# ajgupta93/d4pg-pytorch

Hardware: AMD Instinct MI355X
Metric: learner grad-steps/sec (Pendulum-v1 D4PG) (higher is better)
Workload: dtype fp32; 1 GPU; model=D4PG Pendulum-v1 (obs3/act1, 4x256 MLP actor+critic, 51 atoms), global_batch=64, parallelism=dp1 (one learner per GPU), n_step=5, prioritized_replay=True, replay_capacity=1000000, device=cuda

## Files before the change

d4pg_amd/ops/hip/engine_common.hip:

```cpp

#include <hip/hip_runtime.h>
#include <cstdint>
#include <cstdio>
#include <cstring>
#include <cstdlib>
#include <cmath>
#include <vector>
#include <stdexcept>

#define HIP_CHECK(cmd) do { \
    hipError_t e_ = (cmd); \
    if (e_ != hipSuccess) { \
        char buf[256]; \
        snprintf(buf, sizeof(buf), "HIP error %s at %s:%d", \
                 hipGetErrorString(e_), __FILE__, __LINE__); \
        throw std::runtime_error(buf); \
    } \
} while (0)

namespace d4pg {

__device__ __forceinline__ uint32_t mulhi32(uint32_t a, uint32_t b) {
    return (uint32_t)(((uint64_t)a * b) >> 32);
}

struct Philox4 { uint32_t v[4]; };

__device__ inline Philox4 philox4(uint64_t seed, uint64_t ctr_hi,
                                  uint64_t ctr_lo) {
    uint32_t c0 = (uint32_t)ctr_lo, c1 = (uint32_t)(ctr_lo >> 32);
    uint32_t c2 = (uint32_t)ctr_hi, c3 = (uint32_t)(ctr_hi >> 32);
    uint32_t k0 = (uint32_t)seed, k1 = (uint32_t)(seed >> 32);
    const uint32_t M0 = 0xD2511F53u, M1 = 0xCD9E8D57u;
    const uint32_t W0 = 0x9E3779B9u, W1 = 0xBB67AE85u;
#pragma unroll
    for (int r = 0; r < 10; ++r) {
        uint32_t hi0 = mulhi32(M0, c0), lo0 = M0 * c0;
        uint32_t hi1 = mulhi32(M1, c2), lo1 = M1 * c2;
        uint32_t n0 = hi1 ^ c1 ^ k0, n1 = lo1;
        uint32_t n2 = hi0 ^ c3 ^ k1, n3 = lo0;
        c0 = n0; c1 = n1; c2 = n2; c3 = n3;
        k0 += W0; k1 += W1;
    }
    return {c0, c1, c2, c3};
}

__device__ inline float u01(uint32_t x) {
    return ((float)x + 1.0f) * 2.3283064e-10f;
}


struct LayerDesc {
    int in1, in2, out;
    long w_off, b_off;
};

enum Act { ACT_NONE = 0, ACT_RELU = 1, ACT_TANH = 2, ACT_SOFTMAX = 3 };

struct EngineCfg {
    int obs, act, hidden, atoms, batch;
    long capacity;
    float v_min, v_max, gamma_n, tau, lr_actor, lr_critic;
    float per_alpha, per_beta0, per_eps;
    long per_beta_iters;
    uint64_t seed;
    int is_weighting;
    int prioritized = 1;
    int true_td = 0;
};

struct Counters {
    long long beta_t;
    long long adam_t_actor;
    long long adam_t_critic;
    long long rng_epoch;
    long long size;
    long long pos;
    float max_priority;
    float loss_critic;
    float loss_actor;
};

#define FWD_XMAX 1032

__device__ inline float act_mask(int act, float h) {
    if (act == ACT_RELU) return h > 0.f ? 1.f : 0.f;
    if (act == ACT_TANH) return 1.f - h * h;
    return 1.f;
}

struct NetPtrs { const float *w1, *b1, *w2, *b2, *w3, *b3, *w4, *b4; };

__device__ inline NetPtrs net_ptrs(const float* slab, const LayerDesc* l) {
    return {slab + l[0].w_off, slab + l[0].b_off,
            slab + l[1].w_off, slab + l[1].b_off,
            slab + l[2].w_off, slab + l[2].b_off,
            slab + l[3].w_off, slab + l[3].b_off};
}

struct StepArgs {
    int B, O, A, H, K;
    float v_min, v_max, gamma_n, per_eps, tau, lr_actor, lr_critic;
    float per_alpha, per_beta0, per_beta_iters;
    int is_weighting;
    int prioritized, true_td;
    uint64_t seed;
    long tree_cap;
    long n_actor, n_critic;
    LayerDesc al[4], cl[4];
    float *p_actor, *p_actor_t, *p_critic, *p_critic_t;
    float *g_actor, *g_critic, *m_actor, *v_actor, *m_critic, *v_critic;
    float *rs, *ra, *rr, *rs2, *rd;
    double *sum_tree, *min_tree;
    float *bs, *bs_b, *ba, *br, *bs2, *bd, *bw, *pri;
    long *bidx;
    float *at_h1, *at_h2, *at_h3, *a2;
    float *ct_h1, *ct_h2, *ct_h3, *p_t, *m_proj;
    float *c_h1, *c_h2, *c_h3, *q, *dlog, *d3, *d2, *d1;
    float *pa_h1, *pa_h2, *pa_h3, *a_out;
    float *pc_h1, *pc_h2, *pc_h3, *pq;
    float *pd3, *pd2, *pdh1, *adz, *az1, *az2, *az3;
    Counters* cnt;
    unsigned long long* gbar;
    unsigned long long* tstamp;
    float *da, *pda;
};


}
```

d4pg_amd/ops/hip/engine_persistent.hip:

```cpp

namespace d4pg {

#define PNWG 96
#define PW4 (PNWG / 4)
#define PW3A (PNWG / 3)
#define PW3B (PNWG - 2 * (PNWG / 3))
#define PROWS 4
#define PXMAX 512
#define PWOFF (PROWS * PXMAX)
#define PLDS_FLOATS (2 * 4 * PXMAX + 2 * 64 * 68 + 64)

#define PTIMEW(g, s, i, w) \
    do { if ((int)blockIdx.x == (w) && threadIdx.x == 0 && (s) == pts) \
        (g).tstamp[i] = __builtin_amdgcn_s_memrealtime(); } while (0)
#define PTIME(g, s, i) PTIMEW(g, s, i, 0)

__device__ inline void bar_release() {
    __builtin_amdgcn_fence(__ATOMIC_RELEASE, "agent");
    asm volatile("s_waitcnt vmcnt(0)" ::: "memory");
}
__device__ inline void bar_acquire() {
    __builtin_amdgcn_fence(__ATOMIC_ACQUIRE, "agent");
    asm volatile("s_waitcnt vmcnt(0)" ::: "memory");
}

__device__ inline void p_bar(unsigned long long* gb,
                             unsigned long long& round) {
    __syncthreads();
    round += 1;
    if (threadIdx.x == 0) {
        bar_release();
        int grp = blockIdx.x & 7;
        unsigned long long old = atomicAdd(&gb[grp << 4], 1ull);
        if (old + 1 == round * (PNWG >> 3)) {
            unsigned long long r = atomicAdd(&gb[128], 1ull);
            if (r + 1 == round * 8)
                __hip_atomic_store(&gb[144], round, __ATOMIC_RELEASE,
                                   __HIP_MEMORY_SCOPE_AGENT);
        }
        volatile unsigned long long* f = &gb[144];
        volatile unsigned long long* err = &gb[176];
        long spins = 0;
        while (*f < round) {
            if (++spins > (1L << 26)) {
                atomicAdd((unsigned long long*)err, 1ull);
                break;
            }
            if (spins < 48) __builtin_amdgcn_s_sleep(2);
            else {
                __builtin_amdgcn_s_sleep(32);
                if ((spins & 63) == 0 && *err) break;
            }
        }
        bar_acquire();
    }
    __syncthreads();
}

__device__ inline void q_bar(unsigned long long* qc,
                             unsigned long long& qround) {
    __syncthreads();
    qround += 4;
    if (threadIdx.x == 0) {
        bar_release();
        atomicAdd(qc, 1ull);
        volatile unsigned long long* f = qc;
        long spins = 0;
        while (*f < qround) {
            if (++spins > (1L << 26)) break;
            __builtin_amdgcn_s_sleep(1);
        }
        bar_acquire();
    }
    __syncthreads();
}

__device__ inline void t_bar(unsigned long long* tc,
                             unsigned long long& trnd, int members) {
    __syncthreads();
    trnd += members;
    if (threadIdx.x == 0) {
        bar_release();
        atomicAdd(tc, 1ull);
        volatile unsigned long long* f = tc;
        long spins = 0;
        while (*f < trnd) {
            if (++spins > (1L << 26)) break;
            __builtin_amdgcn_s_sleep(1);
        }
        bar_acquire();
    }
    __syncthreads();
}

__device__ __noinline__ void p_fwd(float* lds, const float* x1, const float* x2,
                             const float* wt, const float* bias, float* y,
                             int B, int in1, int in2, int out, int act_kind,
                             int wg_rel, int nwg) {
    int in_total = in1 + in2;
    int in_pad = (in_total + 3) & ~3;
    int nrt = (B + PROWS - 1) / PROWS;
    int nct = (out + 63) / 64;
    int ntiles = nrt * nct;
    int tid = threadIdx.x;
    for (int t = wg_rel; t < ntiles; t += nwg) {
        int r0 = (t / nct) * PROWS, c0 = (t % nct) * 64;
        int kk16 = tid >> 6, cc16 = tid & 63;
        float wreg[16];
        int nfull = in_total >> 6;
        auto preload = [&](int kc) {
#pragma unroll
            for (int u = 0; u < 16; ++u) {
                int gk = kc + kk16 + 4 * u, gc = c0 + cc16;
                wreg[u] = (gc < out)
                    ? wt[(long)gk * out + gc] : 0.f;
            }
        };
        if (nfull > 0) preload(0);
        {
            int tot = PROWS * in_pad;
            for (int base = 0; base < tot; base += 256 * 8) {
                float tmp[8];
#pragma unroll
                for (int u = 0; u < 8; ++u) {
                    int e = base + u * 256 + tid;
                    float v = 0.f;
                    if (e < tot) {
                        int rr_ = e / in_pad, kk = e % in_pad;
                        int gb = r0 + rr_;
                        if (gb < B && kk < in_total)
                            v = (kk < in1)
                                ? x1[(long)gb * in1 + kk]
                                : x2[(long)gb * in2 + (kk - in1)];
                    }
                    tmp[u] = v;
                }
#pragma unroll
                for (int u = 0; u < 8; ++u) {
                    int e = base + u * 256 + tid;
                    if (e < tot) lds[e] = tmp[u];
                }
            }
        }
        __syncthreads();
        int rq = tid >> 6, c = tid & 63;
        int o = c0 + c;
        int r = r0 + rq;
        float acc = 0.f;
        float* ws = lds + PWOFF;
        const float* xr = lds + rq * in_pad;
        for (int ch = 0; ch < nfull; ++ch) {
            int kc = ch << 6;
            float wb[16];
#pragma unroll
            for (int u = 0; u < 16; ++u) wb[u] = wreg[u];
            if (kc + 64 < (nfull << 6)) preload(kc + 64);
#pragma unroll
            for (int u = 0; u < 16; ++u)
                ws[cc16 * 68 + kk16 + 4 * u] = wb[u];
            __syncthreads();
            if (o < out) {
                const float* wcol = ws + c * 68;
#pragma unroll
                for (int k = 0; k < 64; k += 4) {
                    float4 wv = *reinterpret_cast<const float4*>(wcol + k);
                    float4 xv = *reinterpret_cast<const float4*>(
                        xr + kc + k);
                    acc += xv.x * wv.x;
                    acc += xv.y * wv.y;
                    acc += xv.z * wv.z;
                    acc += xv.w * wv.w;
                }
            }
            __syncthreads();
        }
        int kc = nfull << 6, klen = in_total - kc;
        if (klen > 0) {
            for (int e = tid; e < (klen << 6); e += 256) {
                int kk = e >> 6, cc = e & 63;
                int gc = c0 + cc;
                ws[cc * 68 + kk] = (gc < out)
                    ? wt[(long)(kc + kk) * out + gc] : 0.f;
            }
            __syncthreads();
            if (o < out) {
                for (int k = 0; k < klen; ++k)
                    acc += xr[kc + k] * ws[c * 68 + k];
            }
            __syncthreads();
        }
        if (act_kind == ACT_SOFTMAX) {
            float v = (o < out) ? acc + bias[o] : -INFINITY;
            float mx = v;
            for (int s = 32; s > 0; s >>= 1)
                mx = fmaxf(mx, __shfl_xor(mx, s, 64));
            float e = (o < out) ? __expf(v - mx) : 0.f;
            float sum = e;
            for (int s = 32; s > 0; s >>= 1) sum += __shfl_xor(sum, s, 64);
            if (r < B && o < out) y[(long)r * out + o] = e / sum;
        } else if (r < B && o < out) {
            float v = acc + bias[o];
            if (act_kind == ACT_RELU) v = fmaxf(v, 0.f);
            else if (act_kind == ACT_TANH) v = tanhf(v);
            y[(long)r * out + o] = v;
        }
        __syncthreads();
    }
}

__device__ inline void p_bwd_dx(float* lds, const float* dz, const float* wt,
                                int in_lo, int in_hi, int out, int B,
                                const float* hprev, int prev_act, float* dx,
                                int wg_rel, int nwg) {
    int span = in_hi - in_lo;
    int nrt = (B + PROWS - 1) / PROWS;
    int nit = (span + 63) / 64;
    int ntiles = nrt * nit;
    int tid = threadIdx.x;
    for (int t = wg_rel; t < ntiles; t += nwg) {
        int r0 = (t / nit) * PROWS, i0 = in_lo + (t % nit) * 64;
        int oo16 = tid & 3;
        int ii16 = tid >> 2;
        float wreg[16];
        int gi_ld = i0 + ii16;
        int nfull = out >> 6;
        auto preload = [&](int oc) {
#pragma unroll
            for (int u = 0; u < 16; ++u) {
                int go = oc + oo16 + 4 * u;
                wreg[u] = (gi_ld < in_hi)
                    ? wt[(long)gi_ld * out + go] : 0.f;
            }
        };
        if (nfull > 0) preload(0);
        int out_pad = (out + 3) & ~3;
        {
            int tot = PROWS * out_pad;
            for (int base = 0; base < tot; base += 256 * 8) {
                float tmp[8];
#pragma unroll
                for (int u = 0; u < 8; ++u) {
                    int e = base + u * 256 + tid;
                    float v = 0.f;
                    if (e < tot) {
                        int rr_ = e / out_pad, oo = e % out_pad;
                        int gb = r0 + rr_;
                        if (gb < B && oo < out)
                            v = dz[(long)gb * out + oo];
                    }
                    tmp[u] = v;
                }
#pragma unroll
                for (int u = 0; u < 8; ++u) {
                    int e = base + u * 256 + tid;
                    if (e < tot) lds[e] = tmp[u];
                }
            }
        }
        __syncthreads();
        int rq = tid >> 6, c = tid & 63;
        int i = i0 + c;
        int r = r0 + rq;
        float acc = 0.f;
        float* ws = lds + PWOFF;
        const float* zr = lds + rq * out_pad;
        for (int ch = 0; ch < nfull; ++ch) {
            int oc = ch << 6;
            float wb[16];
#pragma unroll
            for (int u = 0; u < 16; ++u) wb[u] = wreg[u];
            if (oc + 64 < (nfull << 6)) preload(oc + 64);
#pragma unroll
            for (int u = 0; u < 16; ++u)
                ws[ii16 * 68 + oo16 + 4 * u] = wb[u];
            __syncthreads();
            if (i < in_hi) {
                const float* wrow = ws + c * 68;
#pragma unroll
                for (int o = 0; o < 64; o += 4) {
                    float4 wv = *reinterpret_cast<const float4*>(wrow + o);
                    float4 zv = *reinterpret_cast<const float4*>(
                        zr + oc + o);
                    acc += zv.x * wv.x;
                    acc += zv.y * wv.y;
                    acc += zv.z * wv.z;
                    acc += zv.w * wv.w;
                }
            }
            __syncthreads();
        }
        int oc = nfull << 6, olen = out - oc;
        if (olen > 0) {
            for (int e = tid; e < 4096; e += 256) {
                int ii = e >> 6, oo = e & 63;
                int gi = i0 + ii;
                ws[ii * 68 + oo] = (gi < in_hi && oo < olen)
                    ? wt[(long)gi * out + (oc + oo)] : 0.f;
            }
            __syncthreads();
            if (i < in_hi) {
                for (int o = 0; o < olen; ++o)
                    acc += zr[oc + o] * ws[c * 68 + o];
            }
            __syncthreads();
        }
        if (r < B && i < in_hi) {
            long rel = (long)r * span + (i - in_lo);
            float m_ = hprev ? act_mask(prev_act, hprev[rel]) : 1.f;
            dx[rel] = acc * m_;
        }
        __syncthreads();
    }
}

__device__ __noinline__ void p_dw2(float* lds, const float* dz,
                                   const float* x1, const float* x2,
                                   float* dwt, float* dbias,
                                   int B, int in1, int in2, int out,
                                   int wg_rel, int nwg) {
    int in_total = in1 + in2;
    int nti = (in_total + 63) >> 6, nto = (out + 63) >> 6;
    int ntiles = nti * nto;
    float* xs = lds;
    float* zs = lds + 64 * 68;
    int tid = threadIdx.x;
    int ig = tid >> 4, og = tid & 15;
    for (int t = wg_rel; t < ntiles; t += nwg) {
        int i0 = (t / nto) << 6, o0 = (t % nto) << 6;
        float acc[4][4] = {};
        float accb[4] = {};
        for (int bc = 0; bc < B; bc += 64) {
            float tx[16], tz[16];
#pragma unroll
            for (int u = 0; u < 16; ++u) {
                int e = u * 256 + tid;
                int bb = e >> 6, ii = e & 63;
                int gb = bc + bb, gi = i0 + ii;
                float xv = 0.f;
                if (gb < B && gi < in_total)
                    xv = (gi < in1) ? x1[(long)gb * in1 + gi]
                                    : x2[(long)gb * in2 + (gi - in1)];
                tx[u] = xv;
                int go = o0 + ii;
                tz[u] = (gb < B && go < out)
                    ? dz[(long)gb * out + go] : 0.f;
            }
#pragma unroll
            for (int u = 0; u < 16; ++u) {
                int e = u * 256 + tid;
                int bb = e >> 6, ii = e & 63;
                xs[bb * 68 + ii] = tx[u];
                zs[bb * 68 + ii] = tz[u];
            }
            __syncthreads();
            int blim = min(64, B - bc);
            for (int b = 0; b < blim; ++b) {
                float4 xq = *reinterpret_cast<const float4*>(
                    xs + b * 68 + ig * 4);
                float4 zq = *reinterpret_cast<const float4*>(
                    zs + b * 68 + og * 4);
                float xv0 = xq.x, xv1 = xq.y, xv2 = xq.z, xv3 = xq.w;
                float zv0 = zq.x, zv1 = zq.y, zv2 = zq.z, zv3 = zq.w;
                acc[0][0] += xv0 * zv0; acc[0][1] += xv0 * zv1;
                acc[0][2] += xv0 * zv2; acc[0][3] += xv0 * zv3;
                acc[1][0] += xv1 * zv0; acc[1][1] += xv1 * zv1;
                acc[1][2] += xv1 * zv2; acc[1][3] += xv1 * zv3;
                acc[2][0] += xv2 * zv0; acc[2][1] += xv2 * zv1;
                acc[2][2] += xv2 * zv2; acc[2][3] += xv2 * zv3;
                acc[3][0] += xv3 * zv0; acc[3][1] += xv3 * zv1;
                acc[3][2] += xv3 * zv2; acc[3][3] += xv3 * zv3;
                if (ig == 0 && i0 == 0) {
                    accb[0] += zv0; accb[1] += zv1;
                    accb[2] += zv2; accb[3] += zv3;
                }
            }
            __syncthreads();
        }
#pragma unroll
        for (int a = 0; a < 4; ++a) {
            int gi = i0 + ig * 4 + a;
            if (gi >= in_total) continue;
#pragma unroll
            for (int bb = 0; bb < 4; ++bb) {
                int go = o0 + og * 4 + bb;
                if (go < out) dwt[(long)gi * out + go] = acc[a][bb];
            }
        }
        if (ig == 0 && i0 == 0 && dbias) {
#pragma unroll
            for (int bb = 0; bb < 4; ++bb) {
                int go = o0 + og * 4 + bb;
                if (go < out) dbias[go] = accb[bb];
            }
        }
    }
}

__device__ inline void p_adam_lerp(float* __restrict__ p,
                                   const float* __restrict__ gr,
                                   float* __restrict__ m,
                                   float* __restrict__ v,
                                   float* __restrict__ tgt_slab, long n,
                                   float lr, float tau, long long t,
                                   int nwg = PNWG) {
    const float b1 = 0.9f, b2 = 0.999f, eps = 1e-8f;
    AdamBias bc = adam_bias(b1, b2, t);
    long stride = (long)nwg * 256;
    long i0 = (long)blockIdx.x * 256 + threadIdx.x;
    for (long base = i0; base < n; base += stride * 4) {
        float gi_[4], mi_[4], vi_[4], pi_[4], ti_[4];
#pragma unroll
        for (int u = 0; u < 4; ++u) {
            long i = base + u * stride;
            bool ok = i < n;
            gi_[u] = ok ? gr[i] : 0.f;
            mi_[u] = ok ? m[i] : 0.f;
            vi_[u] = ok ? v[i] : 0.f;
            pi_[u] = ok ? p[i] : 0.f;
            ti_[u] = ok ? tgt_slab[i] : 0.f;
        }
#pragma unroll
        for (int u = 0; u < 4; ++u) {
            long i = base + u * stride;
            if (i >= n) continue;
            float gi = gi_[u];
            float mi = b1 * mi_[u] + (1.f - b1) * gi;
            float vi = b2 * vi_[u] + (1.f - b2) * gi * gi;
            m[i] = mi; v[i] = vi;
            float pn = pi_[u] - lr * (mi / bc.bc1)
                                   / (sqrtf(vi / bc.bc2) + eps);
            p[i] = pn;
            tgt_slab[i] = ti_[u] + tau * (pn - ti_[u]);
        }
    }
}

__device__ inline void p_sample(const StepArgs& g, int wg0,
                                long long epoch, long long beta_t,
                                float* bs_out) {
    int probe = ((int)blockIdx.x - wg0) * 4 + (threadIdx.x >> 6);
    int lane = threadIdx.x & 63;
    if (probe >= g.B) return;
    sample_probe<true>(g, bs_out, probe, lane, epoch, beta_t);
}

__device__ inline void p_project_ce(const StepArgs& g, float* lds,
                                    int row_base = -1) {
    int wid = threadIdx.x >> 6, lane = threadIdx.x & 63;
    int row = (row_base < 0 ? (int)blockIdx.x * 4 : row_base) + wid;
    if (row >= g.B) return;
    int K = g.K;
    float* mrow = lds + wid * 64;
    float p = (lane < K) ? g.p_t[(long)row * K + lane] : 0.f;
    c51_project_row(mrow, p, g.br[row], g.bd[row], g.v_min, g.v_max,
                    g.gamma_n, K, lane);
    float qv = 0.f, mv = 0.f;
    if (lane < K) {
        g.m_proj[(long)row * K + lane] = mrow[lane];
        qv = g.q[(long)row * K + lane];
        mv = mrow[lane];
    }
    float scale = (g.is_weighting && g.bw) ? g.bw[row] : 1.f;
    CeRow r = ce_grad_row(mv, qv, scale, g.B);
    if (lane < K) g.dlog[(long)row * K + lane] = r.dz;
    float pri = ce_priority_row(mv, qv, r.dot,
                                c51_atom(g.v_min, g.v_max, K, lane),
                                g.true_td, g.per_eps);
    if (lane == 0) {
        g.pri[row] = pri;
        atomicAdd(&g.cnt->loss_critic, scale * r.ce / (float)g.B);
    }
}

__device__ inline void p_bwd_dx_narrow(const StepArgs& g, const float* dz,
                                       const float* wt, int in_lo,
                                       int in_hi, int out,
                                       const float* ymask, float* dx,
                                       int row_base = -1) {
    int row = (row_base < 0 ? (int)blockIdx.x * 4 : row_base)
              + (threadIdx.x >> 6);
    int lane = threadIdx.x & 63;
    if (row >= g.B) return;
    int span = in_hi - in_lo;
    for (int j = 0; j < span; ++j) {
        const float* wrow = wt + (long)(in_lo + j) * out;
        float acc = 0.f;
        for (int o = lane; o < out; o += 64)
            acc += dz[(long)row * out + o] * wrow[o];
        for (int s = 32; s > 0; s >>= 1) acc += __shfl_xor(acc, s, 64);
        if (lane == 0) {
            float y = ymask[(long)row * span + j];
            dx[(long)row * span + j] = acc * (1.f - y * y);
        }
    }
}

__device__ inline void p_policy_grad(const StepArgs& g,
                                     int row_base = -1) {
    int row = (row_base < 0 ? (int)blockIdx.x * 4 : row_base)
              + (threadIdx.x >> 6);
    int lane = threadIdx.x & 63;
    if (row >= g.B) return;
    int K = g.K;
    float qv = (lane < K) ? g.pq[(long)row * K + lane] : 0.f;
    float e;
    float dz = policy_grad_row(qv, c51_atom(g.v_min, g.v_max, K, lane), g.B,
                               e);
    if (lane < K) g.pd3[(long)row * K + lane] = dz;
    if (lane == 0) atomicAdd(&g.cnt->loss_actor, -e / (float)g.B);
}

__device__ inline void p_per_update(const StepArgs& g, int owner_wg) {
    if ((int)blockIdx.x != owner_wg || !g.prioritized) return;
    per_write_leaves(g.sum_tree, g.min_tree, g.tree_cap, g.bidx, g.pri, g.B,
                     g.per_alpha, g.cnt);
    per_repair_paths(g.sum_tree, g.min_tree, g.tree_cap, g.B, 256,
                     [&](int i) { return g.tree_cap + g.bidx[i]; });
}

__global__ void __launch_bounds__(256, 1)
k_step_persistent(StepArgs g, int nsteps) {
    __shared__ float lds[PLDS_FLOATS];
    unsigned long long tgt = g.gbar[160];
    unsigned long long* ctr = g.gbar;
    int wg = blockIdx.x;
    unsigned long long qrnd = ctr[192 + ((wg >> 2) << 4)];
    NetPtrs a = net_ptrs(g.p_actor, g.al);
    NetPtrs at = net_ptrs(g.p_actor_t, g.al);
    NetPtrs c = net_ptrs(g.p_critic, g.cl);
    NetPtrs ct = net_ptrs(g.p_critic_t, g.cl);
    const int O = g.O, A = g.A, H = g.H, K = g.K, B = g.B;

    const long long bt0 = g.cnt->beta_t;
    const long long ep0 = g.cnt->rng_epoch;
    const long long ta0 = g.cnt->adam_t_actor;
    const long long tc0 = g.cnt->adam_t_critic;
    const int QW = ((B + 3) / 4) * 4;
    const bool otail = (QW + 32 <= PNWG) && (B <= 128);
    unsigned long long trnd = ctr[1280];
    const int pts = nsteps > 1 ? 1 : 0;

    for (int s = 0; s < nsteps; ++s) {
        float* bs_cur = ((bt0 + s) & 1) ? g.bs_b : g.bs;
        float* bs_nxt = ((bt0 + s) & 1) ? g.bs : g.bs_b;
               PTIME(g, s, 0);
        const bool pipe = otail && s > 0;
        if (!pipe) {
            if (s == 0 || B > (PNWG - PNWG * 3 / 4) * 4) {
                p_sample(g, 0, ep0 + s, bt0 + s, bs_cur);
                p_bar(ctr, tgt);
            }
            PTIME(g, s, 1);
            if (wg < PW4)
                p_fwd(lds, g.bs2, nullptr, at.w1, at.b1, g.at_h1, B, O, 0,
                      H, ACT_RELU, wg, PW4);
            else if (wg < 2 * PW4)
                p_fwd(lds, g.bs2, nullptr, ct.w1, ct.b1, g.ct_h1, B, O, 0,
                      H, ACT_RELU, wg - PW4, PW4);
            else if (wg < 3 * PW4)
                p_fwd(lds, bs_cur, nullptr, c.w1, c.b1, g.c_h1, B, O, 0, H,
                      ACT_RELU, wg - 2 * PW4, PW4);
            else
                p_fwd(lds, bs_cur, nullptr, a.w1, a.b1, g.pa_h1, B, O, 0, H,
                      ACT_RELU, wg - 3 * PW4, PW4);
            p_bar(ctr, tgt); PTIME(g, s, 2);
            if (wg < PW3A)
                p_fwd(lds, g.at_h1, nullptr, at.w2, at.b2, g.at_h2, B, H, 0,
                      H, ACT_NONE, wg, PW3A);
            else if (wg < 2 * PW3A)
                p_fwd(lds, g.c_h1, g.ba, c.w2, c.b2, g.c_h2, B, H, A, H,
                      ACT_RELU, wg - PW3A, PW3A);
            else
                p_fwd(lds, g.pa_h1, nullptr, a.w2, a.b2, g.pa_h2, B, H, 0,
                      H, ACT_NONE, wg - 2 * PW3A, PW3B);
            p_bar(ctr, tgt); PTIME(g, s, 3);
            if (wg < PW3A)
                p_fwd(lds, g.at_h2, nullptr, at.w3, at.b3, g.at_h3, B, H, 0,
                      H, ACT_RELU, wg, PW3A);
            else if (wg < 2 * PW3A)
                p_fwd(lds, g.c_h2, nullptr, c.w3, c.b3, g.c_h3, B, H, 0, H,
                      ACT_RELU, wg - PW3A, PW3A);
            else
                p_fwd(lds, g.pa_h2, nullptr, a.w3, a.b3, g.pa_h3, B, H, 0,
                      H, ACT_RELU, wg - 2 * PW3A, PW3B);
            p_bar(ctr, tgt); PTIME(g, s, 4);
            if (wg < PW3A)
                p_fwd(lds, g.at_h3, nullptr, at.w4, at.b4, g.a2, B, H, 0, A,
                      ACT_TANH, wg, PW3A);
            else if (wg < 2 * PW3A)
                p_fwd(lds, g.c_h3, nullptr, c.w4, c.b4, g.q, B, H, 0, K,
                      ACT_SOFTMAX, wg - PW3A, PW3A);
            else
                p_fwd(lds, g.pa_h3, nullptr, a.w4, a.b4, g.a_out, B, H, 0,
                      A, ACT_TANH, wg - 2 * PW3A, PW3B);
            if (wg == PNWG - 1 && threadIdx.x == 0) {
                g.cnt->loss_critic = 0.f;
                g.cnt->loss_actor = 0.f;
            }
            p_bar(ctr, tgt);
        } else {
            PTIME(g, s, 1); PTIME(g, s, 2); PTIME(g, s, 3); PTIME(g, s, 4);
        }
        PTIME(g, s, 5);
        {
            int q = wg >> 2, m = wg & 3;
            unsigned long long* qc = ctr + 192 + (q << 4);
            if (pipe && wg >= QW && wg < QW + 32) {
                p_fwd(lds, bs_cur, nullptr, a.w1, a.b1, g.pa_h1, B, O, 0, H,
                      ACT_RELU, wg - QW, 32);
                t_bar(ctr + 1280, trnd, 32);
                p_fwd(lds, g.pa_h1, nullptr, a.w2, a.b2, g.pa_h2, B, H, 0,
                      H, ACT_NONE, wg - QW, 32);
                t_bar(ctr + 1280, trnd, 32);
                p_fwd(lds, g.pa_h2, nullptr, a.w3, a.b3, g.pa_h3, B, H, 0,
                      H, ACT_RELU, wg - QW, 32);
                t_bar(ctr + 1280, trnd, 32);
                p_fwd(lds, g.pa_h3, nullptr, a.w4, a.b4, g.a_out, B, H, 0,
                      A, ACT_TANH, wg - QW, 32);
                PTIMEW(g, s, 53, QW);
            }
            for (int rg = q; rg < (B + 3) / 4; rg += PNWG / 4) {
                long r0 = (long)rg * 4;
                int nb = min(4, B - (int)r0);
                if (pipe) {
                    p_fwd(lds, g.bs2 + r0 * O, nullptr, at.w1, at.b1,
                          g.at_h1 + r0 * H, nb, O, 0, H, ACT_RELU, m, 4);
                    q_bar(qc, qrnd);
                    p_fwd(lds, g.at_h1 + r0 * H, nullptr, at.w2, at.b2,
                          g.at_h2 + r0 * H, nb, H, 0, H, ACT_NONE, m, 4);
                    q_bar(qc, qrnd);
                    p_fwd(lds, g.at_h2 + r0 * H, nullptr, at.w3, at.b3,
                          g.at_h3 + r0 * H, nb, H, 0, H, ACT_RELU, m, 4);
                    q_bar(qc, qrnd);
                    p_fwd(lds, g.at_h3 + r0 * H, nullptr, at.w4, at.b4,
                          g.a2 + r0 * A, nb, H, 0, A, ACT_TANH, m, 4);
                    q_bar(qc, qrnd); PTIME(g, s, 54);
                }
                p_fwd(lds, g.ct_h1 + r0 * H, g.a2 + r0 * A, ct.w2, ct.b2,
                      g.ct_h2 + r0 * H, nb, H, A, H, ACT_RELU, m, 4);
                q_bar(qc, qrnd);
                p_fwd(lds, g.ct_h2 + r0 * H, nullptr, ct.w3, ct.b3,
                      g.ct_h3 + r0 * H, nb, H, 0, H, ACT_RELU, m, 4);
                q_bar(qc, qrnd);
                p_fwd(lds, g.ct_h3 + r0 * H, nullptr, ct.w4, ct.b4,
                      g.p_t + r0 * K, nb, H, 0, K, ACT_SOFTMAX, m, 4);
                if (m == 0)
                    p_project_ce(g, lds, (int)r0);
                PTIME(g, s, 55);
            }
        }
        p_bar(ctr, tgt);
        PTIME(g, s, 6); PTIME(g, s, 7); PTIME(g, s, 8); PTIME(g, s, 9);
        {
            int q = wg >> 2, m = wg & 3;
            unsigned long long* qc = ctr + 192 + (q << 4);
            if (otail) p_per_update(g, QW);
            for (int rg = q; rg < (B + 3) / 4; rg += PNWG / 4) {
                long r0 = (long)rg * 4;
                int nb = min(4, B - (int)r0);
                p_bwd_dx(lds, g.dlog + r0 * K, c.w4, 0, H, K, nb,
                         g.c_h3 + r0 * H, ACT_RELU, g.d3 + r0 * H, m, 4);
                q_bar(qc, qrnd);
                p_bwd_dx(lds, g.d3 + r0 * H, c.w3, 0, H, H, nb,
                         g.c_h2 + r0 * H, ACT_RELU, g.d2 + r0 * H, m, 4);
                q_bar(qc, qrnd);
                p_bwd_dx(lds, g.d2 + r0 * H, c.w2, 0, H, H, nb,
                         g.c_h1 + r0 * H, ACT_RELU, g.d1 + r0 * H, m, 4);
            }
        }
        p_bar(ctr, tgt);
        PTIME(g, s, 10); PTIME(g, s, 11); PTIME(g, s, 12);
        if (wg < PNWG / 16)
            p_dw2(lds, g.d1, bs_cur, nullptr, g.g_critic + g.cl[0].w_off,
                 g.g_critic + g.cl[0].b_off, B, O, 0, H, wg, PNWG / 16);
        else if (wg < PNWG / 2)
            p_dw2(lds, g.d2, g.c_h1, g.ba, g.g_critic + g.cl[1].w_off,
                 g.g_critic + g.cl[1].b_off, B, H, A, H, wg - PNWG / 16,
                 PNWG / 2 - PNWG / 16);
        else if (wg < PNWG * 7 / 8)
            p_dw2(lds, g.d3, g.c_h2, nullptr, g.g_critic + g.cl[2].w_off,
                 g.g_critic + g.cl[2].b_off, B, H, 0, H, wg - PNWG / 2,
                 PNWG * 7 / 8 - PNWG / 2);
        else
            p_dw2(lds, g.dlog, g.c_h3, nullptr, g.g_critic + g.cl[3].w_off,
                 g.g_critic + g.cl[3].b_off, B, H, 0, K, wg - PNWG * 7 / 8,
                 PNWG - PNWG * 7 / 8);
        p_bar(ctr, tgt); PTIME(g, s, 13);
        p_adam_lerp(g.p_critic, g.g_critic, g.m_critic, g.v_critic,
                    g.p_critic_t, g.n_critic, g.lr_critic, g.tau,
                    tc0 + s);
        p_bar(ctr, tgt); PTIME(g, s, 14);
        {
            int q = wg >> 2, m = wg & 3;
            unsigned long long* qc = ctr + 192 + (q << 4);
            if (otail && wg >= QW && wg < QW + 32) {
                if (s + 1 < nsteps) {
                    p_sample(g, QW, ep0 + s + 1, bt0 + s + 1, bs_nxt);
                    t_bar(ctr + 1280, trnd, 32);
                    p_fwd(lds, g.bs2, nullptr, ct.w1, ct.b1, g.ct_h1, B,
                          O, 0, H, ACT_RELU, wg - QW, 32);
                    p_fwd(lds, bs_nxt, nullptr, c.w1, c.b1, g.c_h1, B, O,
                          0, H, ACT_RELU, wg - QW, 32);
                    t_bar(ctr + 1280, trnd, 32);
                    p_fwd(lds, g.c_h1, g.ba, c.w2, c.b2, g.c_h2, B, H, A,
                          H, ACT_RELU, wg - QW, 32);
                    t_bar(ctr + 1280, trnd, 32);
                    p_fwd(lds, g.c_h2, nullptr, c.w3, c.b3, g.c_h3, B, H,
                          0, H, ACT_RELU, wg - QW, 32);
                    t_bar(ctr + 1280, trnd, 32);
                    p_fwd(lds, g.c_h3, nullptr, c.w4, c.b4, g.q, B, H, 0,
                          K, ACT_SOFTMAX, wg - QW, 32);
                }
                PTIMEW(g, s, 52, QW);
            }
            for (int rg = q; rg < (B + 3) / 4; rg += PNWG / 4) {
                long r0 = (long)rg * 4;
                int nb = min(4, B - (int)r0);
                PTIME(g, s, 40);
                p_fwd(lds, bs_cur + r0 * O, nullptr, c.w1, c.b1,
                      g.pc_h1 + r0 * H, nb, O, 0, H, ACT_RELU, m, 4);
                q_bar(qc, qrnd); PTIME(g, s, 41);
                p_fwd(lds, g.pc_h1 + r0 * H, g.a_out + r0 * A, c.w2, c.b2,
                      g.pc_h2 + r0 * H, nb, H, A, H, ACT_RELU, m, 4);
                q_bar(qc, qrnd); PTIME(g, s, 42);
                p_fwd(lds, g.pc_h2 + r0 * H, nullptr, c.w3, c.b3,
                      g.pc_h3 + r0 * H, nb, H, 0, H, ACT_RELU, m, 4);
                q_bar(qc, qrnd); PTIME(g, s, 43);
                p_fwd(lds, g.pc_h3 + r0 * H, nullptr, c.w4, c.b4,
                      g.pq + r0 * K, nb, H, 0, K, ACT_SOFTMAX, m, 4);
                if (m == 0)
                    p_policy_grad(g, (int)r0);
                q_bar(qc, qrnd); PTIME(g, s, 44);
                p_bwd_dx(lds, g.pd3 + r0 * K, c.w4, 0, H, K, nb,
                         g.pc_h3 + r0 * H, ACT_RELU, g.pd2 + r0 * H, m, 4);
                q_bar(qc, qrnd); PTIME(g, s, 45);
                p_bwd_dx(lds, g.pd2 + r0 * H, c.w3, 0, H, H, nb,
                         g.pc_h2 + r0 * H, ACT_RELU, g.pdh1 + r0 * H,
                         m, 4);
                q_bar(qc, qrnd); PTIME(g, s, 46);
                if (m == 0)
                    p_bwd_dx_narrow(g, g.pdh1, c.w2, H, H + A, H,
                                    g.a_out, g.adz, (int)r0);
                q_bar(qc, qrnd); PTIME(g, s, 47);
                p_bwd_dx(lds, g.adz + r0 * A, a.w4, 0, H, A, nb,
                         g.pa_h3 + r0 * H, ACT_RELU, g.az3 + r0 * H, m, 4);
                q_bar(qc, qrnd); PTIME(g, s, 48);
                p_bwd_dx(lds, g.az3 + r0 * H, a.w3, 0, H, H, nb,
                         nullptr, ACT_NONE, g.az2 + r0 * H, m, 4);
                q_bar(qc, qrnd); PTIME(g, s, 49);
                p_bwd_dx(lds, g.az2 + r0 * H, a.w2, 0, H, H, nb,
                         g.pa_h1 + r0 * H, ACT_RELU, g.az1 + r0 * H, m, 4);
                PTIME(g, s, 51);
            }
        }
        p_bar(ctr, tgt);
        PTIME(g, s, 15); PTIME(g, s, 16); PTIME(g, s, 17);
        PTIME(g, s, 18); PTIME(g, s, 19); PTIME(g, s, 20);
        PTIME(g, s, 21); PTIME(g, s, 22); PTIME(g, s, 23);
        PTIME(g, s, 24); PTIME(g, s, 25);
        if (wg < PNWG / 16)
            p_dw2(lds, g.az1, bs_cur, nullptr, g.g_actor + g.al[0].w_off,
                 g.g_actor + g.al[0].b_off, B, O, 0, H, wg, PNWG / 16);
        else if (wg < PNWG * 15 / 32)
            p_dw2(lds, g.az2, g.pa_h1, nullptr, g.g_actor + g.al[1].w_off,
                 g.g_actor + g.al[1].b_off, B, H, 0, H, wg - PNWG / 16,
                 PNWG * 15 / 32 - PNWG / 16);
        else if (wg < PNWG * 7 / 8)
            p_dw2(lds, g.az3, g.pa_h2, nullptr, g.g_actor + g.al[2].w_off,
                 g.g_actor + g.al[2].b_off, B, H, 0, H, wg - PNWG * 15 / 32,
                 PNWG * 7 / 8 - PNWG * 15 / 32);
        else if (wg < PNWG - 2)
            p_dw2(lds, g.adz, g.pa_h3, nullptr, g.g_actor + g.al[3].w_off,
                 g.g_actor + g.al[3].b_off, B, H, 0, A, wg - PNWG * 7 / 8,
                 PNWG - 2 - PNWG * 7 / 8);
        else if (!otail && wg == PNWG - 1)
            p_per_update(g, PNWG - 1);
        p_bar(ctr, tgt); PTIME(g, s, 26);
        {
            int anw = otail ? PNWG : PNWG * 3 / 4;
            if (wg < anw)
                p_adam_lerp(g.p_actor, g.g_actor, g.m_actor, g.v_actor,
                            g.p_actor_t, g.n_actor, g.lr_actor, g.tau,
                            ta0 + s, anw);
            else if (s + 1 < nsteps && B <= (PNWG - PNWG * 3 / 4) * 4)
                p_sample(g, PNWG * 3 / 4, ep0 + s + 1, bt0 + s + 1, bs_nxt);
            if (otail && s + 1 < nsteps && wg == PNWG - 1
                && threadIdx.x == 0) {
                g.cnt->loss_critic = 0.f;
                g.cnt->loss_actor = 0.f;
            }
        }
        p_bar(ctr, tgt); PTIME(g, s, 27); PTIME(g, s, 28);
    }
    if (wg == 0 && threadIdx.x == 0) {
        g.cnt->beta_t = bt0 + nsteps;
        g.cnt->rng_epoch = ep0 + nsteps;
        g.cnt->adam_t_actor = ta0 + nsteps;
        g.cnt->adam_t_critic = tc0 + nsteps;
        g.gbar[160] = tgt;
    }
}

}
```

d4pg_amd/ops/hip/engine_rowmath.hip:

```cpp

namespace d4pg {

__device__ __forceinline__ float softmax_wave(float v, bool valid) {
    float mx = valid ? v : -INFINITY;
    for (int s = 32; s > 0; s >>= 1) mx = fmaxf(mx, __shfl_xor(mx, s, 64));
    float e = valid ? __expf(v - mx) : 0.f;
    float sum = e;
    for (int s = 32; s > 0; s >>= 1) sum += __shfl_xor(sum, s, 64);
    return e / sum;
}

__device__ __forceinline__ float c51_bins(float tz, float v_min, float delta,
                                          int K, int& l, int& u) {
    float b = fminf((tz - v_min) / delta, (float)(K - 1));
    l = (int)floorf(b);
    u = (int)ceilf(b);
    if (l == u) { if (u > 0) l -= 1; else u += 1; }
    return b;
}

__device__ __forceinline__ float c51_atom(float v_min, float v_max, int K,
                                          int lane) {
    float delta = (v_max - v_min) / (K - 1);
    return v_min + lane * delta;
}

__device__ __forceinline__ void c51_project_row(float* mrow, float p, float r,
                                                float d, float v_min,
                                                float v_max, float gamma_n,
                                                int K, int lane) {
    mrow[lane] = 0.f;
    __builtin_amdgcn_wave_barrier();
    if (lane < K) {
        float delta = (v_max - v_min) / (K - 1);
        float z = v_min + lane * delta;
        float tz = r + gamma_n * (1.f - d) * z;
        tz = fminf(v_max, fmaxf(v_min, tz));
        int l, u;
        float b = c51_bins(tz, v_min, delta, K, l, u);
        atomicAdd(&mrow[l], p * ((float)u - b));
        atomicAdd(&mrow[u], p * (b - (float)l));
    }
    __builtin_amdgcn_wave_barrier();
}

struct CeRow { float dz, dot, ce; };

__device__ __forceinline__ CeRow ce_grad_row(float mv, float qv, float scale,
                                             int B) {
    float dot = mv * qv;
    float ce = -mv * __logf(qv + 1e-10f);
    for (int s = 32; s > 0; s >>= 1) {
        dot += __shfl_xor(dot, s, 64);
        ce += __shfl_xor(ce, s, 64);
    }
    return {scale * (qv - mv) / (float)B, dot, ce};
}

__device__ __forceinline__ float ce_priority_row(float mv, float qv,
                                                 float dot, float z,
                                                 int true_td, float per_eps) {
    if (!true_td) return dot + per_eps;
    float em = mv * z, eq = qv * z;
    for (int s = 32; s > 0; s >>= 1) {
        em += __shfl_xor(em, s, 64);
        eq += __shfl_xor(eq, s, 64);
    }
    return fabsf(em - eq) + per_eps;
}

__device__ __forceinline__ float policy_grad_row(float qv, float z, int B,
                                                 float& e) {
    e = qv * z;
    for (int s = 32; s > 0; s >>= 1) e += __shfl_xor(e, s, 64);
    return -qv * (z - e) / (float)B;
}

template <bool NT>
__device__ __forceinline__ long per_descend(const double* sum_tree,
                                            long tree_cap, double mass) {
    auto ld = [&](long i, bool deep) {
        return (NT && deep) ? __builtin_nontemporal_load(&sum_tree[i])
                            : sum_tree[i];
    };
    long node = 1;
    while (node < tree_cap / 2) {
        long gb = 4 * node;
        bool deep = gb >= 16384;
        double g0 = ld(gb, deep), g1 = ld(gb + 1, deep),
               g2 = ld(gb + 2, deep);
        double s01 = g0 + g1;
        if (mass <= s01) {
            if (mass <= g0) node = gb;
            else { mass -= g0; node = gb + 1; }
        } else {
            mass -= s01;
            if (mass <= g2) node = gb + 2;
            else { mass -= g2; node = gb + 3; }
        }
    }
    if (node < tree_cap) {
        double ls = ld(2 * node, node >= 16384);
        if (mass > ls) { mass -= ls; node = 2 * node + 1; }
        else           { node = 2 * node; }
    }
    return node;
}

__device__ __forceinline__ float per_beta(long long beta_t, float beta0,
                                          float beta_iters) {
    float frac = fminf((float)((double)beta_t / beta_iters), 1.0f);
    return beta0 + frac * (1.0f - beta0);
}

__device__ __forceinline__ float per_is_weight(double p, double p_min,
                                               long long n, float beta) {
    double max_w = pow(p_min * (double)n, (double)-beta);
    return (float)(pow(p * (double)n, (double)-beta) / max_w);
}

template <bool NT>
__device__ __forceinline__ void sample_gather_row(const StepArgs& g,
                                                  float* bs_out, int probe,
                                                  int lane, long idx) {
    auto ld = [](const float* p) {
        return NT ? __builtin_nontemporal_load(p) : *p;
    };
    idx = __shfl(idx, 0, 64);
    for (int k = lane; k < g.O; k += 64) {
        bs_out[(long)probe * g.O + k] = ld(&g.rs[idx * g.O + k]);
        g.bs2[(long)probe * g.O + k] = ld(&g.rs2[idx * g.O + k]);
    }
    for (int k = lane; k < g.A; k += 64)
        g.ba[(long)probe * g.A + k] = ld(&g.ra[idx * g.A + k]);
}

template <bool NT>
__device__ __forceinline__ void per_sample_probe(const StepArgs& g,
                                                 float* bs_out, int probe,
                                                 int lane, long long epoch,
                                                 long long beta_t) {
    long long n = g.cnt->size;
    double total = g.sum_tree[1];
    float beta = per_beta(beta_t, g.per_beta0, g.per_beta_iters);
    long idx = 0;
    if (lane == 0) {
        Philox4 r = philox4(g.seed, (uint64_t)epoch, (uint64_t)probe);
        double mass = (double)u01(r.v[0]) * total;
        idx = per_descend<NT>(g.sum_tree, g.tree_cap, mass) - g.tree_cap;
        if (idx >= n) idx = n - 1;
        g.bidx[probe] = idx;
        g.bw[probe] = per_is_weight(g.sum_tree[g.tree_cap + idx] / total,
                                    g.min_tree[1] / total, n, beta);
        g.br[probe] = g.rr[idx];
        g.bd[probe] = g.rd[idx];
    }
    sample_gather_row<NT>(g, bs_out, probe, lane, idx);
}

template <bool NT>
__device__ __forceinline__ void uniform_sample_probe(const StepArgs& g,
                                                     float* bs_out, int probe,
                                                     int lane, long long epoch,
                                                     long long ) {
    long idx = 0;
    if (lane == 0) {
        unsigned long long n = (unsigned long long)g.cnt->size;
        Philox4 r = philox4(g.seed, (uint64_t)epoch, (uint64_t)probe);
        unsigned long long x = ((unsigned long long)r.v[0] << 32) | r.v[1];
        idx = (long)__umul64hi(x, n);
        g.bidx[probe] = idx;
        g.bw[probe] = 1.0f;
        g.br[probe] = g.rr[idx];
        g.bd[probe] = g.rd[idx];
    }
    sample_gather_row<NT>(g, bs_out, probe, lane, idx);
}

template <bool NT>
__device__ __forceinline__ void sample_probe(const StepArgs& g, float* bs_out,
                                             int probe, int lane,
                                             long long epoch,
                                             long long beta_t) {
    if (g.prioritized)
        per_sample_probe<NT>(g, bs_out, probe, lane, epoch, beta_t);
    else
        uniform_sample_probe<NT>(g, bs_out, probe, lane, epoch, beta_t);
}

__device__ __forceinline__ double per_leaf_value(float p, float alpha) {
    return pow((double)p, (double)alpha);
}

__device__ __forceinline__ void per_write_leaves(double* sum_tree,
                                                 double* min_tree,
                                                 long tree_cap,
                                                 const long* idx,
                                                 const float* pri, int B,
                                                 float alpha, Counters* cnt) {
    int tid = threadIdx.x;
    float local_max = 0.f;
    for (int i = tid; i < B; i += 256) {
        float p = pri[i];
        double pa = per_leaf_value(p, alpha);
        long leaf = tree_cap + idx[i];
        sum_tree[leaf] = pa;
        min_tree[leaf] = pa;
        local_max = fmaxf(local_max, p);
    }
    __shared__ float smax[256];
    smax[tid] = local_max;
    __syncthreads();
    for (int s = 128; s > 0; s >>= 1) {
        if (tid < s) smax[tid] = fmaxf(smax[tid], smax[tid + s]);
        __syncthreads();
    }
    if (tid == 0)
        cnt->max_priority = fmaxf(cnt->max_priority, smax[0]);
    __syncthreads();
}

template <typename LeafOf>
__device__ __forceinline__ void per_repair_paths(double* sum_tree,
                                                 double* min_tree,
                                                 long tree_cap, int n,
                                                 int nthr, LeafOf leaf_of) {
    long levels = 0;
    for (long c = tree_cap; c > 1; c >>= 1) ++levels;
    for (long lv = 0; lv < levels; ++lv) {
        for (int i = threadIdx.x; i < n; i += nthr) {
            long node = leaf_of(i) >> (lv + 1);
            if (node >= 1) {
                sum_tree[node] = sum_tree[2 * node] + sum_tree[2 * node + 1];
                min_tree[node] = fmin(min_tree[2 * node],
                                      min_tree[2 * node + 1]);
            }
        }
        __syncthreads();
    }
}

__device__ __forceinline__ void tick_counters(Counters* cnt) {
    if (threadIdx.x == 0) {
        cnt->beta_t += 1;
        cnt->adam_t_actor += 1;
        cnt->adam_t_critic += 1;
        cnt->rng_epoch += 1;
    }
}

struct AdamBias { float bc1, bc2; };

__device__ __forceinline__ AdamBias adam_bias(float b1, float b2,
                                              long long t) {
    return {1.f - __powf(b1, (float)t), 1.f - __powf(b2, (float)t)};
}

}
```

Measured before the change: 5045 grad_steps/s.

## Replace fenced sub-barriers with relaxed agent-scope atomics on inter-workgroup activations

```diff
diff --git a/d4pg_amd/ops/hip/engine_common.hip b/d4pg_amd/ops/hip/engine_common.hip
--- a/d4pg_amd/ops/hip/engine_common.hip
+++ b/d4pg_amd/ops/hip/engine_common.hip
@@ -89,6 +89,16 @@
     return 1.f;
 }
 
+typedef __attribute__((address_space(1))) float gfloat;
+__device__ __forceinline__ void st_wt(float* p, float v) {
+    __hip_atomic_store((gfloat*)p, v, __ATOMIC_RELAXED,
+                       __HIP_MEMORY_SCOPE_AGENT);
+}
+__device__ __forceinline__ float ld_wt(const float* p) {
+    return __hip_atomic_load((const gfloat*)p, __ATOMIC_RELAXED,
+                             __HIP_MEMORY_SCOPE_AGENT);
+}
+
 struct NetPtrs { const float *w1, *b1, *w2, *b2, *w3, *b3, *w4, *b4; };
 
 __device__ inline NetPtrs net_ptrs(const float* slab, const LayerDesc* l) {
diff --git a/d4pg_amd/ops/hip/engine_persistent.hip b/d4pg_amd/ops/hip/engine_persistent.hip
--- a/d4pg_amd/ops/hip/engine_persistent.hip
+++ b/d4pg_amd/ops/hip/engine_persistent.hip
@@ -22,6 +22,25 @@
 __device__ inline void bar_acquire() {
     __builtin_amdgcn_fence(__ATOMIC_ACQUIRE, "agent");
     asm volatile("s_waitcnt vmcnt(0)" ::: "memory");
+}
+
+typedef __attribute__((address_space(1))) unsigned long long gu64;
+
+__device__ __forceinline__ void bar_handoff(unsigned long long* ctr,
+                                            unsigned long long want) {
+    asm volatile("s_waitcnt vmcnt(0)" ::: "memory");
+    __syncthreads();
+    if (threadIdx.x == 0) {
+        atomicAdd(ctr, 1ull);
+        long spins = 0;
+        while (__hip_atomic_load((gu64*)ctr, __ATOMIC_RELAXED,
+                                 __HIP_MEMORY_SCOPE_AGENT) < want) {
+            if (++spins > (1L << 26)) break;
+            __builtin_amdgcn_s_sleep(1);
+        }
+        __builtin_amdgcn_fence(__ATOMIC_ACQUIRE, "wavefront");
+    }
+    __syncthreads();
 }
 
 __device__ inline void p_bar(unsigned long long* gb,
@@ -59,38 +78,14 @@
 
 __device__ inline void q_bar(unsigned long long* qc,
                              unsigned long long& qround) {
-    __syncthreads();
     qround += 4;
-    if (threadIdx.x == 0) {
-        bar_release();
-        atomicAdd(qc, 1ull);
-        volatile unsigned long long* f = qc;
-        long spins = 0;
-        while (*f < qround) {
-            if (++spins > (1L << 26)) break;
-            __builtin_amdgcn_s_sleep(1);
-        }
-        bar_acquire();
-    }
-    __syncthreads();
+    bar_handoff(qc, qround);
 }
 
 __device__ inline void t_bar(unsigned long long* tc,
                              unsigned long long& trnd, int members) {
-    __syncthreads();
     trnd += members;
-    if (threadIdx.x == 0) {
-        bar_release();
-        atomicAdd(tc, 1ull);
-        volatile unsigned long long* f = tc;
-        long spins = 0;
-        while (*f < trnd) {
-            if (++spins > (1L << 26)) break;
-            __builtin_amdgcn_s_sleep(1);
-        }
-        bar_acquire();
-    }
-    __syncthreads();
+    bar_handoff(tc, trnd);
 }
 
 __device__ __noinline__ void p_fwd(float* lds, const float* x1, const float* x2,
@@ -130,8 +125,8 @@
                         int gb = r0 + rr_;
                         if (gb < B && kk < in_total)
                             v = (kk < in1)
-                                ? x1[(long)gb * in1 + kk]
-                                : x2[(long)gb * in2 + (kk - in1)];
+                                ? ld_wt(&x1[(long)gb * in1 + kk])
+                                : ld_wt(&x2[(long)gb * in2 + (kk - in1)]);
                     }
                     tmp[u] = v;
                 }
@@ -197,12 +192,12 @@
             float e = (o < out) ? __expf(v - mx) : 0.f;
             float sum = e;
             for (int s = 32; s > 0; s >>= 1) sum += __shfl_xor(sum, s, 64);
-            if (r < B && o < out) y[(long)r * out + o] = e / sum;
+            if (r < B && o < out) st_wt(&y[(long)r * out + o], e / sum);
         } else if (r < B && o < out) {
             float v = acc + bias[o];
             if (act_kind == ACT_RELU) v = fmaxf(v, 0.f);
             else if (act_kind == ACT_TANH) v = tanhf(v);
-            y[(long)r * out + o] = v;
+            st_wt(&y[(long)r * out + o], v);
         }
         __syncthreads();
     }
@@ -246,7 +241,7 @@
                         int rr_ = e / out_pad, oo = e % out_pad;
                         int gb = r0 + rr_;
                         if (gb < B && oo < out)
-                            v = dz[(long)gb * out + oo];
+                            v = ld_wt(&dz[(long)gb * out + oo]);
                     }
                     tmp[u] = v;
                 }
@@ -306,8 +301,8 @@
         }
         if (r < B && i < in_hi) {
             long rel = (long)r * span + (i - in_lo);
-            float m_ = hprev ? act_mask(prev_act, hprev[rel]) : 1.f;
-            dx[rel] = acc * m_;
+            float m_ = hprev ? act_mask(prev_act, ld_wt(&hprev[rel])) : 1.f;
+            st_wt(&dx[rel], acc * m_);
         }
         __syncthreads();
     }
@@ -451,7 +446,7 @@
     if (row >= g.B) return;
     int K = g.K;
     float* mrow = lds + wid * 64;
-    float p = (lane < K) ? g.p_t[(long)row * K + lane] : 0.f;
+    float p = (lane < K) ? ld_wt(&g.p_t[(long)row * K + lane]) : 0.f;
     c51_project_row(mrow, p, g.br[row], g.bd[row], g.v_min, g.v_max,
                     g.gamma_n, K, lane);
     float qv = 0.f, mv = 0.f;
@@ -486,11 +481,11 @@
         const float* wrow = wt + (long)(in_lo + j) * out;
         float acc = 0.f;
         for (int o = lane; o < out; o += 64)
-            acc += dz[(long)row * out + o] * wrow[o];
+            acc += ld_wt(&dz[(long)row * out + o]) * wrow[o];
         for (int s = 32; s > 0; s >>= 1) acc += __shfl_xor(acc, s, 64);
         if (lane == 0) {
-            float y = ymask[(long)row * span + j];
-            dx[(long)row * span + j] = acc * (1.f - y * y);
+            float y = ld_wt(&ymask[(long)row * span + j]);
+            st_wt(&dx[(long)row * span + j], acc * (1.f - y * y));
         }
     }
 }
@@ -502,11 +497,11 @@
     int lane = threadIdx.x & 63;
     if (row >= g.B) return;
     int K = g.K;
-    float qv = (lane < K) ? g.pq[(long)row * K + lane] : 0.f;
+    float qv = (lane < K) ? ld_wt(&g.pq[(long)row * K + lane]) : 0.f;
     float e;
     float dz = policy_grad_row(qv, c51_atom(g.v_min, g.v_max, K, lane), g.B,
                                e);
-    if (lane < K) g.pd3[(long)row * K + lane] = dz;
+    if (lane < K) st_wt(&g.pd3[(long)row * K + lane], dz);
     if (lane == 0) atomicAdd(&g.cnt->loss_actor, -e / (float)g.B);
 }
 
diff --git a/d4pg_amd/ops/hip/engine_rowmath.hip b/d4pg_amd/ops/hip/engine_rowmath.hip
--- a/d4pg_amd/ops/hip/engine_rowmath.hip
+++ b/d4pg_amd/ops/hip/engine_rowmath.hip
@@ -126,13 +126,16 @@
     auto ld = [](const float* p) {
         return NT ? __builtin_nontemporal_load(p) : *p;
     };
+    auto st = [](float* p, float v) {
+        if (NT) st_wt(p, v); else *p = v;
+    };
     idx = __shfl(idx, 0, 64);
     for (int k = lane; k < g.O; k += 64) {
-        bs_out[(long)probe * g.O + k] = ld(&g.rs[idx * g.O + k]);
-        g.bs2[(long)probe * g.O + k] = ld(&g.rs2[idx * g.O + k]);
+        st(&bs_out[(long)probe * g.O + k], ld(&g.rs[idx * g.O + k]));
+        st(&g.bs2[(long)probe * g.O + k], ld(&g.rs2[idx * g.O + k]));
     }
     for (int k = lane; k < g.A; k += 64)
-        g.ba[(long)probe * g.A + k] = ld(&g.ra[idx * g.A + k]);
+        st(&g.ba[(long)probe * g.A + k], ld(&g.ra[idx * g.A + k]));
 }
 
 template <bool NT>
```

Result: faster. 5461 grad_steps/s (median of 6 runs) (+8.2%).
